# antao97/SegGroup

Hardware: AMD Instinct MI355X
Metric: pseudo-label scenes/sec (150k pts, 1.5k segs) (higher is better)
Workload: dtype f32 (fp32 accumulate; operands split into 2 x fp16 pieces on v_mfma_f32_32x32x16_f16; kNN / FPS scores in exact fp32 order); 1 GPU; 64 distinct synthetic scenes per GPU per step, 150000 pts / 1500 segs each (BASELINE.json configs[2]; configs[1] = the same scene shape, single scene); mode=ins_infer, scenes_in_flight=112, engine=14 groups x 8 scenes per batched launch, weights=tests/golden/weights_g2.npz, parallelism=scene-parallel x1

## Files before the change

include/seggroup_hip.h:

```cpp
#ifndef SEGGROUP_HIP_H
#define SEGGROUP_HIP_H

#include <stddef.h>
#include <stdint.h>

#ifdef __cplusplus
extern "C" {
#endif

#define SG_OK          0
#define SG_EINVAL     -1
#define SG_EHIP       -2
#define SG_ENOMEM     -3
#define SG_ESTALL     -4
#define SG_EUNSUP     -5
#define SG_EINTERNAL  -6

#define SG_MODE_INS_INFER 0
#define SG_MODE_SEM_INFER 1

#define SG_NUM_LABEL_VECTORS 14
#define SG_RANGE_WORDS 256
#define SG_MAX_POINTS (1 << 20)

const char* sg_last_error(void);
int  sg_version(void);
int  sg_device_count(void);
int  sg_selftest_wave_ops(int* h_mismatches, void* stream);
int  sg_selftest_list_insert(int* h_mismatches, void* stream);

size_t sg_contract_ws_bytes(int S);
int sg_contract_point_edges(const int64_t* d_adj, int E, const int32_t* d_seg_of_point, int N, int S,
                            int32_t* d_out_adj, int out_capacity, int32_t* d_out_count,
                            void* d_ws, size_t ws_bytes, void* stream);

int sg_gather_members(const int32_t* d_seg_points, const int32_t* d_seg_off, int S,
                      const int32_t* d_order, const int32_t* d_dst, const int32_t* d_cl,
                      int32_t* d_members, int32_t* d_pos_of_point, int32_t* d_cluster_of_pos,
                      int32_t* d_slot_of_pos, void* stream);

size_t sg_fps_ws_bytes(int N);
int sg_fps_sample(const float* d_data, int N, int ch_in, const int32_t* d_members, const int32_t* d_cl_off, int C,
                  int P, int ch_out, int transform, float* d_samples, int32_t* d_sel,
                  void* d_ws, size_t ws_bytes, void* stream);

size_t sg_mlp1_ws_bytes(int C);
int sg_mlp1_forward(const float* d_samples, int C, const float* d_w, const float* d_gamma, const float* d_beta,
                    float* d_feat, int feat_stride, void* d_ws, size_t ws_bytes, void* stream);

int sg_edge_distance(const float* d_feat, int feat_stride, int D, const int32_t* d_adj, int E,
                     float* d_dist, void* stream);

int sg_group_max_rows(const float* d_rows, int row_stride, int D, const int32_t* d_goff, const int32_t* d_gidx,
                      int G, float* d_out, int out_stride, void* stream);

int sg_segment_max(const float* d_rows, int N, int D, const int32_t* d_cluster_of_pos,
                   float* d_out, int out_stride, int C, void* stream);

size_t sg_center_ws_bytes(int T, int C);
int sg_center_clusters(const float* d_data, int N, const int32_t* d_members, const int32_t* d_cl_off, int C,
                       const int32_t* d_tile_cl, const int32_t* d_tile_lo, const int32_t* d_tile_hi, int T,
                       const int32_t* d_cl_tile_off, float* d_x9m, float* d_xyzw,
                       void* d_ws, size_t ws_bytes, void* stream);

int sg_cluster_knn(const float* d_xyzw, int N, const int32_t* d_cl_off,
                   const int32_t* d_tile_cl, const int32_t* d_tile_lo, const int32_t* d_tile_hi, int T,
                   int k, int pos0, int32_t* d_knn, void* stream);

int sg_segment_boxes(const float* d_data, const int32_t* d_seg_points, const int32_t* d_seg_off, int S,
                     float* d_box, void* stream);
int sg_cluster_knn_pruned(const float* d_xyzw, int N, const int32_t* d_cl_off,
                          const int32_t* d_tile_cl, const int32_t* d_tile_lo, const int32_t* d_tile_hi, int T,
                          const int32_t* d_cl_seg_off, const int32_t* d_order, const int32_t* d_dst,
                          const int32_t* d_seg_off, const float* d_segbox, const int32_t* d_slot_of_pos,
                          int k, int pos0, int32_t* d_knn, void* stream);

size_t sg_segment_sort_ws_bytes(int N);
int sg_segment_sort_boxes(const float* d_data, int N, const int32_t* d_seg_points, const int32_t* d_seg_off,
                          const int32_t* d_seg_of_point, int S, const int32_t* d_seg_chunk_off, int max_seg, float* d_segbox,
                          int32_t* d_sperm, float* d_chunk_box, double* d_seg_sums, void* d_ws, size_t ws_bytes, void* stream);
int sg_layer_layout(const float* d_data, int N, const int32_t* d_seg_points, const int32_t* d_seg_off, const int32_t* d_sperm, int S,
                    const int32_t* d_order, const int32_t* d_dst, const int32_t* d_cl, const float* d_cl_mean, int32_t* d_members,
                    int32_t* d_pos_of_point, int32_t* d_cluster_of_pos, int32_t* d_slot_of_pos, float* d_x9m, float* d_sxyzw,
                    int32_t* d_smpos, float* d_point_rec, int32_t* d_seed_id, unsigned int* d_range_bits, void* stream);
int sg_knn_operands(const float* d_data, const int32_t* d_seg_points, const int32_t* d_seg_off, const int32_t* d_sperm, int S,
                    const int32_t* d_order, const int32_t* d_dst, float* d_sxyzw, int32_t* d_smpos, void* stream);
int sg_cluster_knn_sorted(const float* d_sxyzw, const int32_t* d_smpos, int N, const int32_t* d_cl_off,
                          const int32_t* d_tile_cl, const int32_t* d_tile_lo, const int32_t* d_tile_hi, int T,
                          const int32_t* d_cl_seg_off, const int32_t* d_order, const int32_t* d_dst,
                          const int32_t* d_seg_off, const int32_t* d_seg_chunk_off, const float* d_segbox,
                          const float* d_chunk_box, const int32_t* d_slot_of_pos, int k, int pos0, int32_t* d_knn, void* stream);
int sg_knn_seed_points(const int32_t* d_knn, const int32_t* d_members, int N, int k, int32_t* d_seed, void* stream);
int sg_cluster_knn_seeded(const float* d_sxyzw, const int32_t* d_smpos, int N, const int32_t* d_cl_off,
                          const int32_t* d_tile_cl, const int32_t* d_tile_lo, const int32_t* d_tile_hi, int T,
                          const int32_t* d_cl_seg_off, const int32_t* d_order, const int32_t* d_dst,
                          const int32_t* d_seg_off, const int32_t* d_seg_chunk_off, const float* d_segbox,
                          const float* d_chunk_box, const int32_t* d_slot_of_pos, const int32_t* d_seed,
                          const int32_t* d_seg_prevcl, const int32_t* d_members, const float* d_point_rec,
                          int k, int pos0, int32_t* d_knn, void* stream);

int sg_knn_chunk_table(const int32_t* d_order, const int32_t* d_dst, const int32_t* d_seg_off, const int32_t* d_seg_chunk_off,
                       const float* d_chunk_box, int S, const int32_t* d_slot_chunk0, float* d_cc, void* stream);
int sg_cluster_knn_2pass(const float* d_sxyzw, const int32_t* d_smpos, int N, const int32_t* d_cl_off,
                         const int32_t* d_tile_cl, const int32_t* d_tile_lo, const int32_t* d_tile_hi,
                         const int32_t* d_tile_chunk0, int T, const int32_t* d_cl_chunk_off, const float* d_cc,
                         int k, int pos0, int32_t* d_knn, void* stream);
int sg_cluster_knn_sorted_w(const float* d_sxyzw, const int32_t* d_smpos, int N, const int32_t* d_cl_off,
                            const int32_t* d_tile_cl, const int32_t* d_tile_lo, const int32_t* d_tile_hi, int T,
                            const int32_t* d_cl_seg_off, const int32_t* d_order, const int32_t* d_dst,
                            const int32_t* d_seg_off, const int32_t* d_seg_chunk_off, const float* d_segbox,
                            const float* d_chunk_box, const int32_t* d_slot_of_pos, int k, int pos0, int waves_per_tile,
                            int32_t* d_knn, void* stream);

size_t sg_edgeconv_ws_bytes(int N);
int sg_edgeconv_forward(const float* d_x9m, const int32_t* d_knn, int N, int k, int layers,
                        const float* d_w1, const float* d_g1, const float* d_b1,
                        const float* d_w2, const float* d_g2, const float* d_b2,
                        float* d_out, void* d_ws, size_t ws_bytes, void* stream);
int sg_edgeconv_forward_r(const float* d_x9m, const int32_t* d_knn, int N, int k, int layers, const float* d_w1, const float* d_g1,
                          const float* d_b1, const float* d_w2, const float* d_g2, const float* d_b2, float* d_out, void* d_ws,
                          size_t ws_bytes, unsigned int* d_range_bits, void* stream);
#define SG_EDGECONV_COMPILER_LOOP 1u
int sg_edgeconv_forward_x(const float* d_x9m, const int32_t* d_knn, int N, int k, int layers, const float* d_w1, const float* d_g1,
                          const float* d_b1, const float* d_w2, const float* d_g2, const float* d_b2, float* d_out, void* d_ws,
                          size_t ws_bytes, unsigned int* d_range_bits, unsigned int flags, void* stream);
int sg_edge_range(const float* d_x9m, int N, unsigned int* d_range_bits, void* stream);

size_t sg_gcn_ws_bytes(int S, int D, int E);
int sg_gcn_forward(const float* d_x, int S, int D, const int32_t* d_adj, int E,
                   const int32_t* d_rowptr, const int32_t* d_col, const int32_t* d_eid,
                   const float* d_w, float alpha, float* d_out, void* d_ws, size_t ws_bytes, void* stream);

int sg_export_labels(const int32_t* d_unmap, int V, const int32_t* d_seg_of_point, int N,
                     const int32_t* d_tables, int T, int S, int32_t* d_out, void* stream);

size_t sg_eval_ws_bytes(int max_ins);
int sg_evaluate(const int32_t* d_gt, const int32_t* d_sem_pred, const int32_t* d_ins_pred, int V, int max_ins,
                float* h_iou_sem, float* h_iou_ins, float* h_acc, void* d_ws, size_t ws_bytes, void* stream);

typedef struct sg_partition sg_partition;

sg_partition* sg_partition_create(int S, const int32_t* h_seg_first, const int32_t* h_seg_size,
                                  const int32_t* h_seg_ins, const int32_t* h_seg_sem);
void sg_partition_destroy(sg_partition* p);
int  sg_partition_num_clusters(const sg_partition* p);

int sg_partition_union(sg_partition* p, int seg_root1, int seg_root2);
int sg_partition_find(const sg_partition* p, int s);
int sg_partition_label(const sg_partition* p, int r, int32_t* ins, int32_t* sem, double* npts);

int sg_partition_layer(const sg_partition* p, int32_t* h_root, int32_t* h_cl_of_seg, int32_t* h_order,
                       int32_t* h_cl_seg_off, int32_t* h_cl_pt_off, int32_t* h_dst);

int sg_partition_group_nearby(sg_partition* p, const int32_t* h_root, int C, const float* h_dist,
                              const int32_t* h_adj, int E, float th, uint8_t* h_connected);

int sg_partition_contract(const sg_partition* p, const int32_t* h_root_old, const int32_t* h_adj, int E,
                          const uint8_t* h_keep, int32_t* h_adj_out);

int sg_partition_group_unlabeled(sg_partition* p, int32_t* h_root_io, int* C_io, float* h_feat, int D,
                                 int32_t* h_adj, int* E_io);
int sg_partition_unlabeled_fallback(sg_partition* p, const int32_t* h_root, int C, const float* h_samples, int P);

int sg_partition_export_tables(const sg_partition* p, int32_t* h_seg_tab, int32_t* h_ins_tab, int32_t* h_sem_tab);

typedef struct sg_pipeline sg_pipeline;

typedef struct sg_weights {
    const float* mlp1_w;  const float* mlp1_g;  const float* mlp1_b;
    const float* mlp2_w;  const float* mlp2_g;  const float* mlp2_b;
    const float* gcn2_w;
    const float* mlp3_w1; const float* mlp3_g1; const float* mlp3_b1;
    const float* mlp3_w2; const float* mlp3_g2; const float* mlp3_b2;
    const float* gcn3_w;
} sg_weights;

typedef struct sg_scene {
    int N, S, E0, V;
    const float*   d_data;
    const int64_t* d_adj;
    const int32_t* d_seg_of_point;
    const int32_t* d_seg_points;
    const int32_t* d_seg_off;
    const int32_t* d_unmap;
    const int32_t* d_gt;
    const int32_t* h_seg_first;
    const int32_t* h_seg_size;
    const int32_t* h_seg_ins;
    const int32_t* h_seg_sem;
    const int32_t* h_seg_of_vertex;
} sg_scene;

typedef struct sg_result {
    int32_t* h_labels;
    float iou_sem[80];
    float iou_ins[80];
    float acc[4];
    int32_t trace[5];
    int32_t stalled;
    int32_t used_fallback;
    int32_t* h_tables;
// ... 443 lines not shown
```

seggroup_amd/csrc/kernels_mlp1.hip:

```cpp
#include "engine_ctx.h"
#include "sg_common.h"
#include "knn_device.h"
#include "wave_ops.h"

namespace {

constexpr int K1 = 10;

__device__ inline float knn_score(float xq, float yq, float zq, float xxq, float xc, float yc, float zc, float xxc) {
    const float t = __builtin_fmaf(zq, zc, __builtin_fmaf(yq, yc, xq * xc));
    const float inner = -2.0f * t;
    return ((-xxc) - inner) - xxq;
}

__device__ inline float sqnorm3(float x, float y, float z) { return (x * x + y * y) + z * z; }

__device__ __forceinline__ void mlp1_knn_moments_body(const float* __restrict__ samples, uint8_t* __restrict__ knn,
                                                      double* __restrict__ partial, int c) {
    const int lane = threadIdx.x;
    const float* row = samples + ((size_t)c * 64 + lane) * 6;
    float f[6];
#pragma unroll
    for (int k = 0; k < 6; ++k) f[k] = row[k];
    const float xx = sqnorm3(f[0], f[1], f[2]);

    double kvl[K1];
#pragma unroll
    for (int t = 0; t < K1; ++t) kvl[t] = sgknn::list_empty();
#pragma unroll 8
    for (int j = 0; j < 64; ++j) {
        const float s = knn_score(f[0], f[1], f[2], xx, sgw::bcast(f[0], j), sgw::bcast(f[1], j), sgw::bcast(f[2], j), sgw::bcast(xx, j));
        sgknn::list_insert<K1>(kvl, sgknn::make_key(s, j));
    }
    int bi[K1];
#pragma unroll
    for (int t = 0; t < K1; ++t) bi[t] = sgknn::list_index(kvl[t]);
    uint8_t* ko = knn + ((size_t)c * 64 + lane) * K1;
#pragma unroll
    for (int t = 0; t < K1; ++t) ko[t] = (uint8_t)bi[t];

    double e[K1][6];
    double m0 = 0, m1 = 0, m2 = 0;
#pragma unroll
    for (int t = 0; t < K1; ++t) {
#pragma unroll
        for (int k = 0; k < 6; ++k) e[t][k] = (double)__shfl(f[k], bi[t]);
        m0 += e[t][0]; m1 += e[t][1]; m2 += e[t][2];
    }
    m0 /= K1; m1 /= K1; m2 /= K1;
    double acc[27];
#pragma unroll
    for (int q = 0; q < 27; ++q) acc[q] = 0.0;
#pragma unroll
    for (int t = 0; t < K1; ++t) {
        e[t][0] = (e[t][0] - m0) * 10.0; e[t][1] = (e[t][1] - m1) * 10.0; e[t][2] = (e[t][2] - m2) * 10.0;
        int q = 6;
#pragma unroll
        for (int a = 0; a < 6; ++a) {
            acc[a] += e[t][a];
#pragma unroll
            for (int b = a; b < 6; ++b) acc[q++] += e[t][a] * e[t][b];
        }
    }
#pragma unroll
    for (int q = 0; q < 27; ++q) {
        const double v = sgw::wave_sum(acc[q]);
        if (lane == 0) partial[(size_t)c * 27 + q] = v;
    }
}
__global__ __launch_bounds__(64) void k_mlp1_knn_moments(const float* __restrict__ samples, uint8_t* __restrict__ knn,
                                                         double* __restrict__ partial) {
    mlp1_knn_moments_body(samples, knn, partial, blockIdx.x);
}
__global__ __launch_bounds__(64) void k_mlp1_knn_moments_b(const sg::SlotCtx* __restrict__ cx) {
    const sg::SlotCtx& c = cx[blockIdx.y];
    if ((int)blockIdx.x >= c.S) return;
    mlp1_knn_moments_body(c.samples, c.m1_knn, c.m1_partial, blockIdx.x);
}

__device__ __forceinline__ void mlp1_finalize_body(const double* __restrict__ partial, int C, const float* __restrict__ w,
                                                   const float* __restrict__ gamma, const float* __restrict__ beta,
                                                   float* __restrict__ folded) {
    __shared__ double mom[27];
    {
        const int q = threadIdx.x >> 5, l = threadIdx.x & 31;
        double s = 0.0;
        for (int c = l; c < C; c += 32) s += partial[(size_t)c * 27 + q];
#pragma unroll
        for (int o = 16; o > 0; o >>= 1) s += __shfl_xor(s, o);
        if (l == 0) mom[q] = s / ((double)C * 64.0 * K1);
    }
    __syncthreads();
    const int ch = threadIdx.x;
    if (ch >= 64) return;
    double cov[6][6];
    int q = 6;
    for (int a = 0; a < 6; ++a)
        for (int b = a; b < 6; ++b) { cov[a][b] = cov[b][a] = mom[q] - mom[a] * mom[b]; ++q; }
    double mean = 0.0, var = 0.0;
    for (int a = 0; a < 6; ++a) {
        mean += (double)w[ch * 6 + a] * mom[a];
        for (int b = 0; b < 6; ++b) var += (double)w[ch * 6 + a] * (double)w[ch * 6 + b] * cov[a][b];
    }
    const double a_ = (double)gamma[ch] / sqrt(var + 1e-5);
    for (int k = 0; k < 6; ++k) folded[ch * 6 + k] = (float)(a_ * (double)w[ch * 6 + k]);
    folded[384 + ch] = (float)((double)beta[ch] - a_ * mean);
}
__global__ __launch_bounds__(27 * 32) void k_mlp1_finalize(const double* __restrict__ partial, int C, const float* __restrict__ w,
                                                           const float* __restrict__ gamma, const float* __restrict__ beta,
                                                           float* __restrict__ folded) {
    mlp1_finalize_body(partial, C, w, gamma, beta, folded);
}
__global__ __launch_bounds__(27 * 32) void k_mlp1_finalize_b(const sg::SlotCtx* __restrict__ cx, const float* __restrict__ w,
                                                             const float* __restrict__ gamma, const float* __restrict__ beta) {
    const sg::SlotCtx& c = cx[blockIdx.y];
    mlp1_finalize_body(c.m1_partial, c.S, w, gamma, beta, c.m1_folded);
}

__device__ __forceinline__ void mlp1_apply_body(const float* __restrict__ samples, const uint8_t* __restrict__ knn,
                                                const float* __restrict__ folded, float* __restrict__ feat, int feat_stride, int c) {
    const int lane = threadIdx.x;
    const float* row = samples + ((size_t)c * 64 + lane) * 6;
    float f[6];
#pragma unroll
    for (int k = 0; k < 6; ++k) f[k] = row[k];
    const uint8_t* ki = knn + ((size_t)c * 64 + lane) * K1;
    float e[K1][6];
    double m0 = 0, m1 = 0, m2 = 0;
    double ed[K1][3];
#pragma unroll
    for (int t = 0; t < K1; ++t) {
        const int j = ki[t];
#pragma unroll
        for (int k = 0; k < 6; ++k) e[t][k] = __shfl(f[k], j);
        ed[t][0] = e[t][0]; ed[t][1] = e[t][1]; ed[t][2] = e[t][2];
        m0 += ed[t][0]; m1 += ed[t][1]; m2 += ed[t][2];
    }
    m0 /= K1; m1 /= K1; m2 /= K1;
#pragma unroll
    for (int t = 0; t < K1; ++t) {
        e[t][0] = (float)((ed[t][0] - m0) * 10.0); e[t][1] = (float)((ed[t][1] - m1) * 10.0); e[t][2] = (float)((ed[t][2] - m2) * 10.0);
    }
    float* out = feat + (size_t)c * feat_stride;
    __shared__ float hs[64 * 65];
    __shared__ __attribute__((aligned(8))) float wl[448];
#pragma unroll
    for (int i = 0; i < 7; ++i) {
        const int e_ = lane + 64 * i;
        wl[e_ < 384 ? (e_ % 6) * 64 + e_ / 6 : e_] = folded[e_];
    }
    __builtin_amdgcn_wave_barrier();
    using f32x2 = __attribute__((ext_vector_type(2))) float;
#pragma unroll 2
    for (int ch = 0; ch < 64; ch += 2) {
        f32x2 w[6];
#pragma unroll
        for (int k = 0; k < 6; ++k) w[k] = *reinterpret_cast<const f32x2*>(&wl[k * 64 + ch]);
        const f32x2 b = *reinterpret_cast<const f32x2*>(&wl[384 + ch]);
        float h0 = -INFINITY, h1 = -INFINITY;
#pragma unroll
        for (int t = 0; t < K1; ++t) {
            f32x2 y = b;
#pragma unroll
            for (int k = 0; k < 6; ++k) y = __builtin_elementwise_fma(w[k], f32x2{e[t][k], e[t][k]}, y);
            h0 = fmaxf(h0, y.x);
            h1 = fmaxf(h1, y.y);
        }
        hs[ch * 65 + lane] = fmaxf(h0, 0.2f * h0);
        hs[(ch + 1) * 65 + lane] = fmaxf(h1, 0.2f * h1);
    }
    __builtin_amdgcn_wave_barrier();
    {
        const float* row = hs + lane * 65;
        float mx = -INFINITY;
        double sm = 0.0;
#pragma unroll 8
        for (int i = 0; i < 64; ++i) {
            const float v = row[i];
            mx = fmaxf(mx, v);
            sm += (double)v;
        }
        out[lane] = mx;
        out[64 + lane] = (float)(sm / 64.0);
    }
}
__global__ __launch_bounds__(64) void k_mlp1_apply(const float* __restrict__ samples, const uint8_t* __restrict__ knn,
                                                   const float* __restrict__ folded, float* __restrict__ feat, int feat_stride) {
    mlp1_apply_body(samples, knn, folded, feat, feat_stride, blockIdx.x);
}
__global__ __launch_bounds__(64) void k_mlp1_apply_b(const sg::SlotCtx* __restrict__ cx) {
    const sg::SlotCtx& c = cx[blockIdx.y];
    if ((int)blockIdx.x >= c.S) return;
    mlp1_apply_body(c.samples, c.m1_knn, c.m1_folded, c.feat1, 128, blockIdx.x);
}

__global__ __launch_bounds__(27 * 32) void k_mlp1_bwd_stats(const double* __restrict__ partial, int C, const float* __restrict__ w,
                                                            double* __restrict__ mom_out, float* __restrict__ cst, float* __restrict__ stats_out) {
    __shared__ double mom[27];
    {
        const int q = threadIdx.x >> 5, l = threadIdx.x & 31;
        double s = 0.0;
        for (int c = l; c < C; c += 32) s += partial[(size_t)c * 27 + q];
#pragma unroll
        for (int o = 16; o > 0; o >>= 1) s += __shfl_xor(s, o);
        if (l == 0) { mom[q] = s / ((double)C * 64.0 * K1); mom_out[q] = mom[q]; }
    }
    __syncthreads();
    const int ch = threadIdx.x;
    if (ch >= 64) return;
    double cov[6][6];
    int q = 6;
    for (int a = 0; a < 6; ++a)
        for (int b = a; b < 6; ++b) { cov[a][b] = cov[b][a] = mom[q] - mom[a] * mom[b]; ++q; }
    double mean = 0.0, var = 0.0;
    for (int a = 0; a < 6; ++a) {
        mean += (double)w[ch * 6 + a] * mom[a];
        for (int b = 0; b < 6; ++b) var += (double)w[ch * 6 + a] * (double)w[ch * 6 + b] * cov[a][b];
    }
    var = fmax(var, 0.0);
    cst[ch] = (float)mean;
    cst[64 + ch] = (float)(1.0 / sqrt(var + 1e-5));
    if (stats_out) { stats_out[ch] = (float)mean; stats_out[64 + ch] = (float)var; }
}

__global__ __launch_bounds__(64) void k_mlp1_bwd_rows(const float* __restrict__ samples, const uint8_t* __restrict__ knn, const float* __restrict__ w,
                                                      const float* __restrict__ gamma, const float* __restrict__ beta, const float* __restrict__ cst,
                                                      const float* __restrict__ gfeat, int g_stride, double* __restrict__ rows_partial) {
    const int c = blockIdx.x, lane = threadIdx.x;
    const float* row = samples + ((size_t)c * 64 + lane) * 6;
    float f[6];
#pragma unroll
    for (int k = 0; k < 6; ++k) f[k] = row[k];
    const uint8_t* ki = knn + ((size_t)c * 64 + lane) * K1;
    float e[K1][6];
    double m0 = 0, m1 = 0, m2 = 0;
    double ed[K1][3];
#pragma unroll
    for (int t = 0; t < K1; ++t) {
        const int j = ki[t];
#pragma unroll
        for (int k = 0; k < 6; ++k) e[t][k] = __shfl(f[k], j);
        ed[t][0] = e[t][0]; ed[t][1] = e[t][1]; ed[t][2] = e[t][2];
        m0 += ed[t][0]; m1 += ed[t][1]; m2 += ed[t][2];
    }
    m0 /= K1; m1 /= K1; m2 /= K1;
#pragma unroll
    for (int t = 0; t < K1; ++t) {
        e[t][0] = (float)((ed[t][0] - m0) * 10.0); e[t][1] = (float)((ed[t][1] - m1) * 10.0); e[t][2] = (float)((ed[t][2] - m2) * 10.0);
    }
    const float* g = gfeat + (size_t)c * g_stride;
    double* out = rows_partial + (size_t)c * 512;
    for (int ch = 0; ch < 64; ++ch) {
        const float w0 = w[ch * 6 + 0], w1 = w[ch * 6 + 1], w2 = w[ch * 6 + 2], w3 = w[ch * 6 + 3], w4 = w[ch * 6 + 4], w5 = w[ch * 6 + 5];
        const float mu = cst[ch], inv = cst[64 + ch], ga = gamma[ch], be = beta[ch];
        float best = -INFINITY, bx = 0.f, ba = 0.f;
        float be_[6] = {0.f, 0.f, 0.f, 0.f, 0.f, 0.f};
#pragma unroll
        for (int t = 0; t < K1; ++t) {
            float y = w0 * e[t][0];
            y = __builtin_fmaf(w1, e[t][1], y); y = __builtin_fmaf(w2, e[t][2], y);
            y = __builtin_fmaf(w3, e[t][3], y); y = __builtin_fmaf(w4, e[t][4], y); y = __builtin_fmaf(w5, e[t][5], y);
            const float xh = (y - mu) * inv;
            const float a = xh * ga + be;
            const float h = fmaxf(a, 0.2f * a);
            if (h > best) {
                best = h; bx = xh; ba = a;
#pragma unroll
                for (int k = 0; k < 6; ++k) be_[k] = e[t][k];
            }
        }
        float mv = best;
        int mi = lane;
        sgw::wave_argmax(mv, mi);
        const float dh = (lane == mi ? g[ch] : 0.f) + g[64 + ch] * (1.0f / 64.0f);
        const double da = (double)(dh * (ba > 0.f ? 1.f : 0.2f));
        const double v[8] = {da, da * (double)bx, da * (double)be_[0], da * (double)be_[1], da * (double)be_[2], da * (double)be_[3],
                             da * (double)be_[4], da * (double)be_[5]};
#pragma unroll
        for (int q = 0; q < 8; ++q) {
            const double r = sgw::wave_sum(v[q]);
            if (lane == 0) out[ch * 8 + q] = r;
        }
    }
}

__global__ __launch_bounds__(512) void k_mlp1_bwd_fold(const double* __restrict__ rows_partial, int nparts, int C, const double* __restrict__ mom,
                                                       const float* __restrict__ w, const float* __restrict__ gamma, const float* __restrict__ cst,
                                                       float* __restrict__ gw, float* __restrict__ gg, float* __restrict__ gb) {
    __shared__ double acc[512];
    const int t = threadIdx.x;
    double a = 0.0;
    for (int c = 0; c < nparts; ++c) a += rows_partial[(size_t)c * 512 + t];
    acc[t] = a;
    __syncthreads();
    const double rows = (double)C * 64.0 * K1;
    if (t < 64) { gb[t] = (float)acc[t * 8]; gg[t] = (float)acc[t * 8 + 1]; }
    if (t < 384) {
        const int ch = t / 6, j = t - ch * 6;
        const double inv = (double)cst[64 + ch], mu = (double)cst[ch];
        auto m2 = [&](int p, int q_) {
            const int lo = p < q_ ? p : q_, hi = p < q_ ? q_ : p;
            return mom[6 + lo * 6 - lo * (lo - 1) / 2 + (hi - lo)];
        };
        double wsee = 0.0;
        for (int q_ = 0; q_ < 6; ++q_) wsee += (double)w[ch * 6 + q_] * m2(q_, j);
        const double xe = (wsee - mu * mom[j]) * inv * rows;
        gw[t] = (float)((double)gamma[ch] * inv * (acc[ch * 8 + 2 + j] - acc[ch * 8] / rows * (mom[j] * rows) - acc[ch * 8 + 1] / rows * xe));
    }
}

}

namespace sg {

int b_mlp1(const SlotCtx* d_ctx, const float* d_w, const float* d_g, const float* d_b, const BatchDims& bd, hipStream_t st) {
    if (bd.nslots == 0 || bd.max_S == 0) return SG_OK;
    k_mlp1_knn_moments_b<<<dim3(bd.max_S, bd.nslots), 64, 0, st>>>(d_ctx);
    k_mlp1_finalize_b<<<dim3(1, bd.nslots), 27 * 32, 0, st>>>(d_ctx, d_w, d_g, d_b);
    k_mlp1_apply_b<<<dim3(bd.max_S, bd.nslots), 64, 0, st>>>(d_ctx);
    SG_LAUNCH_CHECK();
    return SG_OK;
}

}

extern "C" {

size_t sg_mlp1_ws_bytes(int C) {
    const size_t c = (size_t)std::max(C, 1);
    return sg::align_up(c * 64 * K1) + sg::align_up(c * 27 * 8) + sg::align_up(448 * 4);
}

int sg_mlp1_forward(const float* d_samples, int C, const float* d_w, const float* d_gamma, const float* d_beta, float* d_feat,
                    int feat_stride, void* d_ws, size_t ws_bytes, void* stream) {
    SG_REQUIRE(C >= 0 && feat_stride >= 128 && d_ws, "sg_mlp1_forward: bad arguments");
    if (C == 0) return SG_OK;
    sg::Carver cv(d_ws, ws_bytes);
    uint8_t* knn = cv.take<uint8_t>((size_t)C * 64 * K1);
    double* partial = cv.take<double>((size_t)C * 27);
    float* folded = cv.take<float>(448);
    if (!cv.ok) return sg::fail(SG_ENOMEM, "sg_mlp1_forward: workspace too small (%zu < %zu)", ws_bytes, sg_mlp1_ws_bytes(C));
    hipStream_t st = sg::as_stream(stream);
    k_mlp1_knn_moments<<<C, 64, 0, st>>>(d_samples, knn, partial);
    k_mlp1_finalize<<<1, 27 * 32, 0, st>>>(partial, C, d_w, d_gamma, d_beta, folded);
    k_mlp1_apply<<<C, 64, 0, st>>>(d_samples, knn, folded, d_feat, feat_stride);
    SG_LAUNCH_CHECK();
    return SG_OK;
}

size_t sg_mlp1_backward_ws_bytes(int C) {
    const size_t c = (size_t)std::max(C, 1);
    return sg::align_up(c * 64 * K1) + sg::align_up(c * 27 * 8) + sg::align_up(c * 512 * 8) + sg::align_up(27 * 8) + sg::align_up(128 * 4) + sg::align_up(512 * 8);
}

int sg_mlp1_backward(const float* d_samples, int C, const float* d_w, const float* d_gamma, const float* d_beta, const float* d_gfeat,
                     int g_stride, float* d_gw, float* d_gg, float* d_gb, float* d_bn_stats, void* d_ws, size_t ws_bytes, void* stream) {
    SG_REQUIRE(C > 0 && g_stride >= 128 && d_samples && d_w && d_gamma && d_beta && d_gfeat && d_gw && d_gg && d_gb && d_ws, "sg_mlp1_backward: bad arguments");
    sg::Carver cv(d_ws, ws_bytes);
    uint8_t* knn = cv.take<uint8_t>((size_t)C * 64 * K1);
    double* partial = cv.take<double>((size_t)C * 27);
    double* rows_partial = cv.take<double>((size_t)C * 512);
    double* mom = cv.take<double>(27);
    float* cst = cv.take<float>(128);
    double* red = cv.take<double>(512);
    if (!cv.ok) return sg::fail(SG_ENOMEM, "sg_mlp1_backward: workspace too small (%zu < %zu)", ws_bytes, sg_mlp1_backward_ws_bytes(C));
    hipStream_t st = sg::as_stream(stream);
    k_mlp1_knn_moments<<<C, 64, 0, st>>>(d_samples, knn, partial);
    k_mlp1_bwd_stats<<<1, 27 * 32, 0, st>>>(partial, C, d_w, mom, cst, d_bn_stats);
    k_mlp1_bwd_rows<<<C, 64, 0, st>>>(d_samples, knn, d_w, d_gamma, d_beta, cst, d_gfeat, g_stride, rows_partial);
    if (int rc = sg::reduce_partials(rows_partial, C, 512, 512, red, st)) return rc;
    k_mlp1_bwd_fold<<<1, 512, 0, st>>>(red, 1, C, mom, d_w, d_gamma, cst, d_gw, d_gg, d_gb);
    SG_LAUNCH_CHECK();
    return SG_OK;
}

}
```

seggroup_amd/hip.py:

```python
from __future__ import annotations

import contextlib
import ctypes as C
import os
import struct
import types
from typing import Optional

_HERE = os.path.dirname(os.path.abspath(__file__))
LIB_PATH = os.environ.get("SEGGROUP_HIP_LIB") or os.path.join(_HERE, "libseggroup_hip.so")
HOST_LIB_OVERRIDE = os.environ.get("SEGGROUP_HIP_HOST_LIB")

SG_OK, SG_EINVAL, SG_EHIP, SG_ENOMEM, SG_ESTALL, SG_EUNSUP, SG_EINTERNAL = 0, -1, -2, -3, -4, -5, -6
MODE_INS_INFER, MODE_SEM_INFER = 0, 1
COLOUR_SEMANTIC, COLOUR_INSTANCE, COLOUR_SEGMENT, COLOUR_GROUPING = 0, 1, 2, 3
NUM_LABEL_VECTORS = 14
KNN_BRUTE, KNN_GRID = 0, 1
KNN_INDEX = {"brute": KNN_BRUTE, "grid": KNN_GRID}
MAX_GRID_POINTS = 1 << 24
MAX_POINTS = 1 << 20
MAX_CLOUD_POINTS = 1 << 27
MAX_RADIUS_PAIRS = 1 << 30


def knn_index(index) -> int:
    if not isinstance(index, str) or index not in KNN_INDEX:
        raise ValueError("index must be 'brute' or 'grid', not %r" % (index,))
    return KNN_INDEX[index]


def knn_cell(cell) -> float:
    c = 0.0 if cell is None else float(cell)
    if not (c >= 0.0) or c == float("inf"):
        raise ValueError("cell must be a finite edge > 0, or None for the library's choice")
    return c
LABEL_NAMES = [f"layer_{l}.{k}" for l in (1, 2, 3, 4) for k in ("seg", "ins", "sem")] + ["final.ins", "final.sem"]

c_f32p = C.POINTER(C.c_float)
c_i32p = C.POINTER(C.c_int32)
c_i64p = C.POINTER(C.c_int64)
c_u8p = C.POINTER(C.c_uint8)
vp = C.c_void_p


class SgError(RuntimeError):
    def __init__(self, code: int, msg: str):
        super().__init__(f"libseggroup_hip error {code}: {msg}")
        self.code = code


class Weights(C.Structure):
    _fields_ = [(n, vp) for n in ("mlp1_w", "mlp1_g", "mlp1_b", "mlp2_w", "mlp2_g", "mlp2_b", "gcn2_w",
                                  "mlp3_w1", "mlp3_g1", "mlp3_b1", "mlp3_w2", "mlp3_g2", "mlp3_b2", "gcn3_w")]


class Scene(C.Structure):
    _fields_ = [("N", C.c_int), ("S", C.c_int), ("E0", C.c_int), ("V", C.c_int),
                ("d_data", vp), ("d_adj", vp), ("d_seg_of_point", vp), ("d_seg_points", vp), ("d_seg_off", vp),
                ("d_unmap", vp), ("d_gt", vp),
                ("h_seg_first", vp), ("h_seg_size", vp), ("h_seg_ins", vp), ("h_seg_sem", vp), ("h_seg_of_vertex", vp)]


class Result(C.Structure):
    _fields_ = [("h_labels", vp), ("iou_sem", C.c_float * 80), ("iou_ins", C.c_float * 80), ("acc", C.c_float * 4),
                ("trace", C.c_int32 * 5), ("stalled", C.c_int32), ("used_fallback", C.c_int32), ("h_tables", vp)]


class Classifier(C.Structure):
    _fields_ = [(n, vp) for n in ("w1", "gamma", "beta", "w2", "b2")]


class Debug(C.Structure):
    _fields_ = [("d_samples1", vp), ("d_feat1", vp), ("d_pointfeat", vp * 2), ("d_knn", vp * 2), ("d_members", vp * 2),
                ("h_gcn", vp * 2), ("h_dist", vp * 3), ("h_adj", vp * 4), ("n_adj", C.c_int32 * 4),
                ("h_feat5", vp), ("h_ins5", vp), ("h_sem5", vp), ("n5", C.c_int32), ("tape", vp), ("d_cat", vp * 2)]


_I, _Z = C.c_int, C.c_size_t
SIGNATURES = {
    "sg_last_error": (C.c_char_p, []),
    "sg_version": (_I, []),
    "sg_device_count": (_I, []),
    "sg_selftest_wave_ops": (_I, [C.POINTER(C.c_int), vp]),
    "sg_selftest_list_insert": (_I, [C.POINTER(C.c_int), vp]),
    "sg_contract_ws_bytes": (_Z, [_I]),
    "sg_contract_point_edges": (_I, [vp, _I, vp, _I, _I, vp, _I, vp, vp, _Z, vp]),
    "sg_gather_members": (_I, [vp, vp, _I, vp, vp, vp, vp, vp, vp, vp, vp]),
    "sg_fps_ws_bytes": (_Z, [_I]),
    "sg_fps_sample": (_I, [vp, _I, _I, vp, vp, _I, _I, _I, _I, vp, vp, vp, _Z, vp]),
    "sg_mlp1_ws_bytes": (_Z, [_I]),
    "sg_mlp1_forward": (_I, [vp, _I, vp, vp, vp, vp, _I, vp, _Z, vp]),
    "sg_edge_distance": (_I, [vp, _I, _I, vp, _I, vp, vp]),
    "sg_group_max_rows": (_I, [vp, _I, _I, vp, vp, _I, vp, _I, vp]),
    "sg_segment_max": (_I, [vp, _I, _I, vp, vp, _I, _I, vp]),
    "sg_center_ws_bytes": (_Z, [_I, _I]),
    "sg_center_clusters": (_I, [vp, _I, vp, vp, _I, vp, vp, vp, _I, vp, vp, vp, vp, _Z, vp]),
    "sg_cluster_knn": (_I, [vp, _I, vp, vp, vp, vp, _I, _I, _I, vp, vp]),
    "sg_segment_boxes": (_I, [vp, vp, vp, _I, vp, vp]),
    "sg_cluster_knn_pruned": (_I, [vp, _I, vp, vp, vp, vp, _I, vp, vp, vp, vp, vp, vp, _I, _I, vp, vp]),
    "sg_segment_sort_ws_bytes": (_Z, [_I]),
    "sg_knn_operands": (_I, [vp, vp, vp, vp, _I, vp, vp, vp, vp, vp]),
    "sg_cluster_knn_sorted": (_I, [vp, vp, _I, vp, vp, vp, vp, _I, vp, vp, vp, vp, vp, vp, vp, vp, _I, _I, vp, vp]),
    "sg_segment_sort_boxes": (_I, [vp, _I, vp, vp, vp, _I, vp, _I, vp, vp, vp, vp, vp, _Z, vp]),
    "sg_layer_layout": (_I, [vp, _I, vp, vp, vp, _I, vp, vp, vp, vp, vp, vp, vp, vp, vp, vp, vp, vp, vp, vp, vp]),
    "sg_cluster_knn_sorted_w": (_I, [vp, vp, _I, vp, vp, vp, vp, _I, vp, vp, vp, vp, vp, vp, vp, vp, _I, _I, _I, vp, vp]),
    "sg_knn_seed_points": (_I, [vp, vp, _I, _I, vp, vp]),
    "sg_cluster_knn_seeded": (_I, [vp, vp, _I, vp, vp, vp, vp, _I, vp, vp, vp, vp, vp, vp, vp, vp, vp, vp, vp, vp, _I, _I, vp, vp]),
    "sg_knn_chunk_table": (_I, [vp, vp, vp, vp, vp, _I, vp, vp, vp]),
    "sg_cluster_knn_2pass": (_I, [vp, vp, _I, vp, vp, vp, vp, vp, _I, vp, vp, _I, _I, vp, vp]),
    "sg_nearest_point_ws_bytes": (_Z, [_I]),
    "sg_nearest_point": (_I, [vp, _I, vp, _I, _I, vp, vp, _Z, vp]),
    "sg_prep_sample_ws_bytes": (_Z, [_I, _I]),
    "sg_prep_sample_points": (_I, [vp, vp, _I, vp, _I, vp, vp, C.POINTER(C.c_int), vp, _Z, vp]),
    "sg_pointcloud_adjacency_ws_bytes": (_Z, [_I, _I]),
    "sg_pointcloud_adjacency": (_I, [vp, _I, _I, _I, vp, C.POINTER(C.c_int), vp, _Z, vp]),
    "sg_mesh_adjacency_ws_bytes": (_Z, [_I]),
    "sg_mesh_adjacency": (_I, [vp, _I, vp, _I, vp, C.POINTER(C.c_int), vp, C.POINTER(C.c_int), vp, _Z, vp]),
    "sg_segment_lists_ws_bytes": (_Z, [_I, _I]),
    "sg_segment_lists": (_I, [vp, _I, vp, _I, vp, vp, vp, C.POINTER(C.c_int), vp, _Z, vp]),
    "sg_write_seg_json": (_I, [C.c_char_p, vp, vp, _I, _I]),
    "sg_overseg_ws_bytes": (_Z, [_I, _I]),
    "sg_overseg_edges": (_I, [vp, _I, vp, _I, vp, vp, vp, vp, C.POINTER(C.c_int), vp, _Z, vp]),
    "sg_overseg_merge": (_I, [vp, vp, _I, _I, C.c_float, _I, vp]),
    "sg_overseg_scan": (_I, [vp, _I, vp, _I, C.c_float, _I, vp, vp, _Z, vp]),
    "sg_overseg_set_timing": (_I, [_I]),
    "sg_overseg_stage_times": (_I, [vp, _I]),
    "sg_overseg_stage_name": (C.c_char_p, [_I]),
    "sg_write_segs_json": (_I, [C.c_char_p, C.c_char_p, vp, _I, C.c_float, _I]),
    "sg_pointcloud_knn_ws_bytes": (_Z, [_I]),
    "sg_pointcloud_knn": (_I, [vp, _I, _I, _I, vp, vp, _Z, vp]),
    "sg_pointcloud_normals": (_I, [vp, _I, vp, _I, vp, vp, vp, _Z, vp]),
    "sg_pcseg_ws_bytes": (_Z, [_I, _I]),
    "sg_pcseg_edges": (_I, [vp, _I, _I, vp, vp, vp, vp, vp, C.POINTER(C.c_int), vp, _Z, vp]),
    "sg_pcseg_scan": (_I, [vp, _I, _I, vp, C.c_float, _I, vp, vp, _Z, vp]),
    "sg_pcseg_set_timing": (_I, [_I]),
    "sg_pcseg_stage_times": (_I, [vp, _I]),
    "sg_pcseg_stage_name": (C.c_char_p, [_I]),
    "sg_cloud_thin_ws_bytes": (_Z, [_I]),
    "sg_cloud_thin": (_I, [vp, _I, _I, C.c_float, vp, vp, C.POINTER(C.c_int), vp, vp, _Z, vp]),
    "sg_cloud_thin_set_timing": (_I, [_I]),
    "sg_cloud_thin_stage_times": (_I, [vp, _I]),
    "sg_cloud_thin_stage_name": (C.c_char_p, [_I]),
    "sg_pointcloud_knn_grid_ws_bytes": (_Z, [_I, _I]),
    "sg_pointcloud_knn_grid": (_I, [vp, _I, _I, _I, C.c_float, vp, vp, _Z, vp]),
    "sg_pointcloud_knn_grid_set_timing": (_I, [_I]),
    "sg_pointcloud_knn_grid_stage_times": (_I, [vp, _I]),
    "sg_pointcloud_knn_grid_stage_name": (C.c_char_p, [_I]),
    "sg_pointcloud_knn_grid_stats": (_I, [vp, _I]),
    "sg_pointcloud_knn_grid_set_tuning": (_I, [_I, _I]),
    "sg_pcseg_ws_bytes_indexed": (_Z, [_I, _I, _I]),
    "sg_pcseg_edges_indexed": (_I, [vp, _I, _I, vp, _I, C.c_float, vp, vp, vp, vp, C.POINTER(C.c_int), vp, _Z, vp]),
    "sg_pcseg_scan_indexed": (_I, [vp, _I, _I, vp, _I, C.c_float, C.c_float, _I, vp, vp, _Z, vp]),
    "sg_nearest_point_grid_ws_bytes": (_Z, [_I, _I]),
    "sg_nearest_point_grid": (_I, [vp, _I, _I, vp, _I, _I, C.c_float, vp, vp, vp, _Z, vp]),
    "sg_nearest_point_grid_set_timing": (_I, [_I]),
    "sg_nearest_point_grid_stage_times": (_I, [vp, _I]),
    "sg_nearest_point_grid_stage_name": (C.c_char_p, [_I]),
    "sg_nearest_point_grid_stats": (_I, [vp, _I]),
    "sg_nearest_point_grid_set_tuning": (_I, [_I, _I]),
    "sg_cloud_knn_cross_grid_ws_bytes": (_Z, [_I, _I, _I]),
    "sg_cloud_knn_cross_grid": (_I, [vp, _I, _I, vp, _I, _I, _I, C.c_float, vp, vp, vp, _Z, vp]),
    "sg_cloud_knn_cross_grid_set_timing": (_I, [_I]),
    "sg_cloud_knn_cross_grid_stage_times": (_I, [vp, _I]),
    "sg_cloud_knn_cross_grid_stage_name": (C.c_char_p, [_I]),
    "sg_cloud_knn_cross_grid_stats": (_I, [vp, _I]),
    "sg_cloud_knn_cross_grid_set_tuning": (_I, [_I, _I]),
    "sg_knn_vote": (_I, [vp, _I, _I, vp, _I, vp, vp, vp, vp, vp]),
    "sg_rigid_apply": (_I, [vp, _I, _I, vp, vp, vp]),
    "sg_align_moments_ws_bytes": (_Z, [_I]),
    "sg_align_moments": (_I, [vp, _I, _I, vp, _I, _I, vp, vp, C.c_float, vp, vp, vp, vp, _Z, vp]),
    "sg_align_solve": (_I, [vp, vp, vp, vp]),
    "sg_align_plane_moments_ws_bytes": (_Z, [_I]),
    "sg_align_plane_moments": (_I, [vp, _I, _I, vp, vp, _I, _I, vp, _I, vp, vp, C.c_float, vp, vp, vp, _Z, vp]),
    "sg_align_plane_solve": (_I, [vp, vp, C.c_double, vp, vp, vp]),
    "sg_fpfh_ws_bytes": (_Z, [_I]),
    "sg_fpfh": (_I, [vp, _I, _I, vp, vp, vp, vp, vp, vp, _Z, vp]),
    "sg_feature_nearest": (_I, [vp, _I, vp, _I, _I, vp, vp, vp]),
    "sg_ransac_ws_bytes": (_Z, [_I, _I]),
    "sg_ransac_count": (_I, [vp, _I, _I, vp, _I, _I, vp, vp, _I, _I, C.c_uint64, vp, C.c_double, C.c_double, C.c_double, vp, C.POINTER(C.c_int),
                             vp, _Z, vp]),
    "sg_ransac_set_tuning": (_I, [_I]),
    "sg_ransac_set_timing": (_I, [_I]),
    "sg_ransac_stage_times": (_I, [vp, _I]),
    "sg_ransac_stage_name": (C.c_char_p, [_I]),
    "sg_triangle_pose": (_I, [vp, vp, vp]),
    "sg_plane_ransac_ws_bytes": (_Z, [_I, _I, _I]),
    "sg_plane_ransac": (_I, [vp, _I, _I, vp, vp, C.c_double, _I, C.c_uint64, vp, C.c_double, C.c_double, C.c_double, vp, vp, C.POINTER(C.c_int),
                             C.POINTER(C.c_int), vp, _Z, vp]),
    "sg_plane_moments_ws_bytes": (_Z, [_I]),
    "sg_plane_moments": (_I, [vp, _I, _I, vp, vp, C.c_double, vp, C.c_double, vp, vp, vp, _Z, vp]),
    "sg_plane_fit": (_I, [vp, vp, vp, vp, vp]),
    "sg_plane_assign_ws_bytes": (_Z, [_I]),
    "sg_plane_assign": (_I, [vp, _I, _I, vp, C.c_double, vp, C.c_double, _I, vp, C.POINTER(C.c_int), vp, _Z, vp]),
    "sg_plane_set_tuning": (_I, [_I]),
    "sg_plane_set_timing": (_I, [_I]),
    "sg_plane_stage_times": (_I, [vp, _I]),
    "sg_plane_stage_name": (C.c_char_p, [_I]),
    "sg_label_index_ws_bytes": (_Z, [_I]),
    "sg_label_index": (_I, [vp, _I, vp, vp, vp, C.POINTER(C.c_int), C.POINTER(C.c_int), vp, _Z, vp]),
    "sg_label_moments_ws_bytes": (_Z, [_I, _I]),
    "sg_label_moments": (_I, [vp, _I, _I, vp, vp, _I, vp, vp, vp, vp, _Z, vp]),
    "sg_label_yaw_boxes_ws_bytes": (_Z, [_I, _I, _I]),
    "sg_label_yaw_boxes": (_I, [vp, _I, _I, vp, vp, _I, vp, _I, vp, vp, vp, vp, _Z, vp]),
    "sg_label_frame_extents_ws_bytes": (_Z, [_I, _I]),
    "sg_label_frame_extents": (_I, [vp, _I, _I, vp, vp, _I, vp, vp, vp, _Z, vp]),
    "sg_box_axes": (_I, [vp, vp, vp]),
    "sg_label_set_timing": (_I, [_I]),
    "sg_label_stage_times": (_I, [vp, _I]),
    "sg_label_stage_name": (C.c_char_p, [_I]),
    "sg_box_iou_ws_bytes": (_Z, [_I, _I, _I]),
    "sg_box_iou": (_I, [vp, _I, vp, _I, vp, vp, _I, vp, C.c_longlong, vp, _Z, vp]),
    "sg_box_best_ws_bytes": (_Z, [_I, _I, _I]),
    "sg_box_best": (_I, [vp, _I, vp, _I, vp, vp, vp, vp, _I, vp, vp, vp, _Z, vp]),
    "sg_box_nms_ws_bytes": (_Z, [_I, _I, C.c_longlong]),
    "sg_box_nms": (_I, [vp, vp, vp, _I, vp, _I, C.c_double, vp, vp, vp, C.c_longlong, vp, _Z, vp]),
    "sg_points_in_boxes_ws_bytes": (_Z, [_I, _I, _I]),
    "sg_points_in_boxes": (_I, [vp, _I, _I, vp, _I, vp, vp, _I, C.c_double, vp, vp, vp, vp, vp, _Z, vp]),
    "sg_components_ws_bytes": (_Z, [_I]),
    "sg_components_edges": (_I, [vp, C.c_longlong, _I, vp, vp, vp, C.POINTER(C.c_int), vp, _Z, vp]),
    "sg_components_faces": (_I, [vp, _I, _I, vp, vp, vp, C.POINTER(C.c_int), vp, _Z, vp]),
    "sg_components_knn": (_I, [vp, _I, vp, _I, _I, C.c_float, vp, vp, vp, C.POINTER(C.c_int), vp, _Z, vp]),
    "sg_components_set_timing": (_I, [_I]),
    "sg_components_stage_times": (_I, [vp, _I]),
    "sg_components_stage_name": (C.c_char_p, [_I]),
    "sg_radius_grid_ws_bytes": (_Z, [_I]),
    "sg_radius_count_grid": (_I, [vp, _I, _I, C.c_float, C.c_float, vp, vp, _Z, vp]),
    "sg_components_radius": (_I, [vp, _I, _I, C.c_float, C.c_float, vp, vp, vp, C.POINTER(C.c_int), vp, _Z, vp]),
    "sg_radius_grid_set_timing": (_I, [_I]),
    "sg_radius_grid_stage_times": (_I, [vp, _I]),
    "sg_radius_grid_stage_name": (C.c_char_p, [_I]),
    "sg_radius_grid_stats": (_I, [vp, _I]),
    "sg_radius_neighbours_ws_bytes": (_Z, [_I, C.c_int64]),
    "sg_radius_neighbours_grid": (_I, [vp, _I, _I, C.c_float, C.c_float, C.c_int64, vp, vp, C.POINTER(C.c_int64), vp, _Z, vp]),
    "sg_pointcloud_normals_csr": (_I, [vp, _I, vp, vp, vp, vp, vp, _Z, vp]),
    "sg_pcseg_ws_bytes_radius": (_Z, [_I, C.c_int64]),
    "sg_pcseg_edges_radius": (_I, [vp, _I, C.c_float, C.c_float, C.c_int64, vp, vp, vp, vp, vp, vp, C.POINTER(C.c_int), C.POINTER(C.c_int64),
                                   vp, _Z, vp]),
    "sg_pcseg_scan_radius": (_I, [vp, _I, C.c_float, C.c_float, C.c_int64, vp, C.c_float, _I, vp, C.POINTER(C.c_int64), vp, _Z, vp]),
    "sg_pcseg_radius_set_timing": (_I, [_I]),
    "sg_pcseg_radius_stage_times": (_I, [vp, _I]),
    "sg_pcseg_radius_stage_name": (C.c_char_p, [_I]),
    "sg_segment_vote_ws_bytes": (_Z, [_I]),
    "sg_segment_rank": (_I, [vp, _I, vp, vp, vp, C.POINTER(C.c_int), vp, _Z, vp]),
    "sg_segment_vote": (_I, [vp, vp, _I, _I] + [vp] * 9 + [C.POINTER(C.c_int), vp, _Z, vp]),
# ... 264 lines not shown
```

Measured before the change: 3552 scenes/s.

## Move MLP1 apply edge-conv matmul onto fp32 MFMA with LDS-staged neighbours

Rewrites the first MLP layer's apply kernel so the per-neighbour 6->64 channel projection runs on v_mfma_f32_32x32x2f32 instead of per-lane VALU FMAs. Neighbour features and folded weights are staged in LDS rather than exchanged with shuffles, and points are handled in two halves of 32 with running max/mean. The old VALU path stays selectable through an env var or a flag on a new forward_x entry point. Launch bounds now request 3 waves per EU, which may limit registers and cause spills, and the MFMA accumulation order can change bits in the fp32 results.

Result: no change. 3577 scenes/s (median of 3 runs) (+0.7%).

```diff
diff --git a/include/seggroup_hip.h b/include/seggroup_hip.h
--- a/include/seggroup_hip.h
+++ b/include/seggroup_hip.h
@@ -47,6 +47,9 @@
 size_t sg_mlp1_ws_bytes(int C);
 int sg_mlp1_forward(const float* d_samples, int C, const float* d_w, const float* d_gamma, const float* d_beta,
                     float* d_feat, int feat_stride, void* d_ws, size_t ws_bytes, void* stream);
+#define SG_MLP1_VALU 1u
+int sg_mlp1_forward_x(const float* d_samples, int C, const float* d_w, const float* d_gamma, const float* d_beta,
+                      float* d_feat, int feat_stride, void* d_ws, size_t ws_bytes, unsigned int flags, void* stream);
 
 int sg_edge_distance(const float* d_feat, int feat_stride, int D, const int32_t* d_adj, int E,
                      float* d_dist, void* stream);
diff --git a/seggroup_amd/csrc/kernels_mlp1.hip b/seggroup_amd/csrc/kernels_mlp1.hip
--- a/seggroup_amd/csrc/kernels_mlp1.hip
+++ b/seggroup_amd/csrc/kernels_mlp1.hip
@@ -117,8 +117,98 @@
     mlp1_finalize_body(c.m1_partial, c.S, w, gamma, beta, c.m1_folded);
 }
 
+using f32x4 = __attribute__((ext_vector_type(4))) float;
+using f32x16 = __attribute__((ext_vector_type(16))) float;
+
 __device__ __forceinline__ void mlp1_apply_body(const float* __restrict__ samples, const uint8_t* __restrict__ knn,
                                                 const float* __restrict__ folded, float* __restrict__ feat, int feat_stride, int c) {
+    const int lane = threadIdx.x, l32 = lane & 31, half = lane >> 5;
+    __shared__ float hs[64 * 33];
+    __shared__ float fs[64 * 7];
+    __shared__ __attribute__((aligned(16))) float wl[448];
+    const float* row = samples + ((size_t)c * 64 + lane) * 6;
+    float f[6], w[7];
+    uint32_t kw[2][5];
+#pragma unroll
+    for (int k = 0; k < 6; ++k) f[k] = row[k];
+#pragma unroll
+    for (int i = 0; i < 7; ++i) w[i] = folded[lane + 64 * i];
+#pragma unroll
+    for (int sh = 0; sh < 2; ++sh) {
+        const uint16_t* kr = reinterpret_cast<const uint16_t*>(knn + ((size_t)c * 64 + 32 * sh + l32) * K1);
+#pragma unroll
+        for (int u = 0; u < 5; ++u) kw[sh][u] = kr[u];
+    }
+#pragma unroll
+    for (int k = 0; k < 6; ++k) fs[lane * 7 + k] = f[k];
+#pragma unroll
+    for (int i = 0; i < 7; ++i) wl[lane + 64 * i] = w[i];
+    __builtin_amdgcn_wave_barrier();
+    float mx = -INFINITY;
+    double sm = 0.0;
+#pragma unroll 1
+    for (int sh = 0; sh < 2; ++sh) {
+        float eb[K1][3];
+        double d0[K1], d1[K1], m0 = 0, m1 = 0;
+#pragma unroll
+        for (int t = 0; t < K1; ++t) {
+            const uint32_t kk = sh ? kw[1][t >> 1] : kw[0][t >> 1];
+            const float* p = fs + (int)((kk >> (8 * (t & 1))) & 255u) * 7 + half;
+            eb[t][0] = p[0]; eb[t][1] = p[2]; eb[t][2] = p[4];
+            d0[t] = eb[t][0]; d1[t] = eb[t][1];
+            m0 += d0[t]; m1 += d1[t];
+        }
+        m0 /= K1; m1 /= K1;
+#pragma unroll
+        for (int t = 0; t < K1; ++t) {
+            eb[t][0] = (float)((d0[t] - m0) * 10.0);
+            const float z = (float)((d1[t] - m1) * 10.0);
+            eb[t][1] = half ? eb[t][1] : z;
+        }
+        if (sh) __builtin_amdgcn_wave_barrier();
+#pragma unroll 1
+        for (int ct = 0; ct < 2; ++ct) {
+            float wa[3];
+            f32x16 shift, hm;
+#pragma unroll
+            for (int m = 0; m < 3; ++m) wa[m] = wl[(32 * ct + l32) * 6 + 2 * m + half];
+#pragma unroll
+            for (int g = 0; g < 4; ++g) {
+                const f32x4 v = *reinterpret_cast<const f32x4*>(&wl[384 + 32 * ct + 8 * g + 4 * half]);
+                shift[4 * g] = v.x; shift[4 * g + 1] = v.y; shift[4 * g + 2] = v.z; shift[4 * g + 3] = v.w;
+            }
+#pragma unroll
+            for (int q = 0; q < 16; ++q) hm[q] = -INFINITY;
+#pragma unroll
+            for (int t = 0; t < K1; ++t) {
+                f32x16 y = shift;
+#pragma unroll
+                for (int m = 0; m < 3; ++m) y = __builtin_amdgcn_mfma_f32_32x32x2f32(wa[m], eb[t][m], y, 0, 0, 0);
+#pragma unroll
+                for (int q = 0; q < 16; ++q) hm[q] = fmaxf(hm[q], y[q]);
+            }
+#pragma unroll
+            for (int q = 0; q < 16; ++q) {
+                const int ch = 32 * ct + (q & 3) + 8 * (q >> 2) + 4 * half;
+                hs[ch * 33 + l32] = fmaxf(hm[q], 0.2f * hm[q]);
+            }
+        }
+        __builtin_amdgcn_wave_barrier();
+        const float* hrow = hs + lane * 33;
+#pragma unroll 8
+        for (int i = 0; i < 32; ++i) {
+            const float v = hrow[i];
+            mx = fmaxf(mx, v);
+            sm += (double)v;
+        }
+    }
+    float* out = feat + (size_t)c * feat_stride;
+    out[lane] = mx;
+    out[64 + lane] = (float)(sm / 64.0);
+}
+
+__device__ __forceinline__ void mlp1_apply_body_valu(const float* __restrict__ samples, const uint8_t* __restrict__ knn,
+                                                     const float* __restrict__ folded, float* __restrict__ feat, int feat_stride, int c) {
     const int lane = threadIdx.x;
     const float* row = samples + ((size_t)c * 64 + lane) * 6;
     float f[6];
@@ -184,15 +274,26 @@
         out[64 + lane] = (float)(sm / 64.0);
     }
 }
-__global__ __launch_bounds__(64) void k_mlp1_apply(const float* __restrict__ samples, const uint8_t* __restrict__ knn,
-                                                   const float* __restrict__ folded, float* __restrict__ feat, int feat_stride) {
+__global__ __launch_bounds__(64, 3) void k_mlp1_apply(const float* __restrict__ samples, const uint8_t* __restrict__ knn,
+                                                      const float* __restrict__ folded, float* __restrict__ feat, int feat_stride) {
     mlp1_apply_body(samples, knn, folded, feat, feat_stride, blockIdx.x);
 }
-__global__ __launch_bounds__(64) void k_mlp1_apply_b(const sg::SlotCtx* __restrict__ cx) {
+__global__ __launch_bounds__(64, 3) void k_mlp1_apply_b(const sg::SlotCtx* __restrict__ cx) {
     const sg::SlotCtx& c = cx[blockIdx.y];
     if ((int)blockIdx.x >= c.S) return;
     mlp1_apply_body(c.samples, c.m1_knn, c.m1_folded, c.feat1, 128, blockIdx.x);
 }
+__global__ __launch_bounds__(64) void k_mlp1_apply_valu(const float* __restrict__ samples, const uint8_t* __restrict__ knn,
+                                                        const float* __restrict__ folded, float* __restrict__ feat, int feat_stride) {
+    mlp1_apply_body_valu(samples, knn, folded, feat, feat_stride, blockIdx.x);
+}
+__global__ __launch_bounds__(64) void k_mlp1_apply_valu_b(const sg::SlotCtx* __restrict__ cx) {
+    const sg::SlotCtx& c = cx[blockIdx.y];
+    if ((int)blockIdx.x >= c.S) return;
+    mlp1_apply_body_valu(c.samples, c.m1_knn, c.m1_folded, c.feat1, 128, blockIdx.x);
+}
+
+const bool g_mlp1_valu = getenv("SG_MLP1_VALU") ? atoi(getenv("SG_MLP1_VALU")) != 0 : false;
 
 __global__ __launch_bounds__(27 * 32) void k_mlp1_bwd_stats(const double* __restrict__ partial, int C, const float* __restrict__ w,
                                                             double* __restrict__ mom_out, float* __restrict__ cst, float* __restrict__ stats_out) {
@@ -317,7 +418,8 @@
     if (bd.nslots == 0 || bd.max_S == 0) return SG_OK;
     k_mlp1_knn_moments_b<<<dim3(bd.max_S, bd.nslots), 64, 0, st>>>(d_ctx);
     k_mlp1_finalize_b<<<dim3(1, bd.nslots), 27 * 32, 0, st>>>(d_ctx, d_w, d_g, d_b);
-    k_mlp1_apply_b<<<dim3(bd.max_S, bd.nslots), 64, 0, st>>>(d_ctx);
+    if (g_mlp1_valu) k_mlp1_apply_valu_b<<<dim3(bd.max_S, bd.nslots), 64, 0, st>>>(d_ctx);
+    else k_mlp1_apply_b<<<dim3(bd.max_S, bd.nslots), 64, 0, st>>>(d_ctx);
     SG_LAUNCH_CHECK();
     return SG_OK;
 }
@@ -331,8 +433,8 @@
     return sg::align_up(c * 64 * K1) + sg::align_up(c * 27 * 8) + sg::align_up(448 * 4);
 }
 
-int sg_mlp1_forward(const float* d_samples, int C, const float* d_w, const float* d_gamma, const float* d_beta, float* d_feat,
-                    int feat_stride, void* d_ws, size_t ws_bytes, void* stream) {
+int sg_mlp1_forward_x(const float* d_samples, int C, const float* d_w, const float* d_gamma, const float* d_beta, float* d_feat,
+                      int feat_stride, void* d_ws, size_t ws_bytes, unsigned int flags, void* stream) {
     SG_REQUIRE(C >= 0 && feat_stride >= 128 && d_ws, "sg_mlp1_forward: bad arguments");
     if (C == 0) return SG_OK;
     sg::Carver cv(d_ws, ws_bytes);
@@ -343,9 +445,15 @@
     hipStream_t st = sg::as_stream(stream);
     k_mlp1_knn_moments<<<C, 64, 0, st>>>(d_samples, knn, partial);
     k_mlp1_finalize<<<1, 27 * 32, 0, st>>>(partial, C, d_w, d_gamma, d_beta, folded);
-    k_mlp1_apply<<<C, 64, 0, st>>>(d_samples, knn, folded, d_feat, feat_stride);
+    if ((flags & SG_MLP1_VALU) || g_mlp1_valu) k_mlp1_apply_valu<<<C, 64, 0, st>>>(d_samples, knn, folded, d_feat, feat_stride);
+    else k_mlp1_apply<<<C, 64, 0, st>>>(d_samples, knn, folded, d_feat, feat_stride);
     SG_LAUNCH_CHECK();
     return SG_OK;
+}
+
+int sg_mlp1_forward(const float* d_samples, int C, const float* d_w, const float* d_gamma, const float* d_beta, float* d_feat,
+                    int feat_stride, void* d_ws, size_t ws_bytes, void* stream) {
+    return sg_mlp1_forward_x(d_samples, C, d_w, d_gamma, d_beta, d_feat, feat_stride, d_ws, ws_bytes, 0u, stream);
 }
 
 size_t sg_mlp1_backward_ws_bytes(int C) {
diff --git a/seggroup_amd/hip.py b/seggroup_amd/hip.py
--- a/seggroup_amd/hip.py
+++ b/seggroup_amd/hip.py
@@ -90,6 +90,7 @@
     "sg_fps_sample": (_I, [vp, _I, _I, vp, vp, _I, _I, _I, _I, vp, vp, vp, _Z, vp]),
     "sg_mlp1_ws_bytes": (_Z, [_I]),
     "sg_mlp1_forward": (_I, [vp, _I, vp, vp, vp, vp, _I, vp, _Z, vp]),
+    "sg_mlp1_forward_x": (_I, [vp, _I, vp, vp, vp, vp, _I, vp, _Z, C.c_uint, vp]),
     "sg_edge_distance": (_I, [vp, _I, _I, vp, _I, vp, vp]),
     "sg_group_max_rows": (_I, [vp, _I, _I, vp, vp, _I, vp, _I, vp]),
     "sg_segment_max": (_I, [vp, _I, _I, vp, vp, _I, _I, vp]),
```
